# voidstrike/FPSG

Hardware: AMD Instinct MI355X
Metric: episodes/sec (+ Chamfer-kernel HBM GB/s in roofline.hbm), 2048-pt clouds, 224x224 images; episode = fwd + Chamfer + bwd, step = E episodes + all-reduce + Adam (higher is better)
Workload: dtype f32

## Files before the change

fpsg_amd/csrc/winograd_dw.hip:

```cpp
#include "fpsg_common.h"

namespace fpsg {
namespace {

constexpr int kDwThreads = 256;

__device__ __forceinline__ void in4(const float (&d)[6], float c0, float (&t)[6]) {
  const float p = fma_rn(-4.0f, d[2], d[4]), q = fma_rn(-4.0f, d[1], d[3]);
  const float r = d[4] - d[2], s = d[3] - d[1];
  t[0] = fma_rn(c0, d[0], fma_rn(-5.0f, d[2], d[4]));
  t[1] = p + q;
  t[2] = p - q;
  t[3] = fma_rn(2.0f, s, r);
  t[4] = fma_rn(-2.0f, s, r);
  t[5] = fma_rn(4.0f, d[1], fma_rn(-5.0f, d[3], d[5]));
}
__device__ __forceinline__ void gout4(const float (&y)[4], float (&r)[6]) {
  const float e = y[0] + y[2], o = y[1] + y[3];
  r[0] = y[0];
  r[1] = e + o;
  r[2] = e - o;
  const float e4 = fma_rn(4.0f, y[2], y[0]), o4 = fma_rn(8.0f, y[3], 2.0f * y[1]);
  r[3] = e4 + o4;
  r[4] = e4 - o4;
  r[5] = y[3];
}

constexpr int kXInstr = 36, kGInstr = 4;
constexpr int kStageFloats = (kXInstr + kGInstr) * 64 * 4;
constexpr int kDma = 10;

template <bool ACT>
__global__ __launch_bounds__(kDwThreads) void wino4_dw_c64_kernel(const float* __restrict__ x, const float* __restrict__ dy,
                                                                  int K, int H, int W, int Th, int Tw, int n_img,
                                                                  long n_steps, int KB, int spr,
                                                                  float* __restrict__ part ,
                                                                  const float* __restrict__ chan,
                                                                  const float* __restrict__ pre_bias) {
  constexpr int C = 64;
  extern __shared__ __attribute__((aligned(16))) float stage[];
  const int tid = threadIdx.x, lane = tid & 63;
  const int wave = __builtin_amdgcn_readfirstlane(tid >> 6);
  const int kk = lane >> 4, col = lane & 15;
  const int i = blockIdx.x;
  const int kb = (i >> 3) % KB;
  const int rg = (i & 7) + 8 * (i / (8 * KB));
  const long s0 = (long)rg * spr;
  const long s1 = (s0 + spr) < n_steps ? (s0 + spr) : n_steps;
  const int cx = wave * 16 + col;
  float* out = part + (((size_t)rg * 36) * K + kb * 16 + 4 * kk) * C + cx;
  if (s0 >= s1) {
#pragma unroll
    for (int xi = 0; xi < 36; ++xi)
#pragma unroll
      for (int r = 0; r < 4; ++r) out[((size_t)xi * K + r) * C] = 0.0f;
    return;
  }
  const __amdgpu_buffer_rsrc_t xrsrc = __builtin_amdgcn_make_buffer_rsrc(
      const_cast<float*>(x), 0, (int)((size_t)n_img * C * H * W * sizeof(float)), 0x00020000);
  const __amdgpu_buffer_rsrc_t grsrc = __builtin_amdgcn_make_buffer_rsrc(
      const_cast<float*>(dy), 0, (int)((size_t)n_img * K * H * W * sizeof(float)), 0x00020000);
  float asc = 1.0f, ash = 0.0f, apb = 0.0f;
  if (ACT) { asc = chan[cx]; ash = chan[C + cx]; apb = pre_bias ? pre_bias[cx] : 0.0f; }

  int fix[kDma];
  int rsel[9];
#pragma unroll
  for (int d = 0; d < 9; ++d) {
    const int p = (wave + 4 * d) * 64 + lane;
    const int r = p / 384, rem = p - r * 384, ch = rem / 6, q = rem - 6 * ch;
    rsel[d] = r;
    fix[d] = ch * H * W + 4 * q - 4;
  }
  {
    const int p = wave * 64 + lane, k = p >> 4, j = ((p & 15) - (k & 7)) & 15;
    fix[9] = ((kb * 16 + k) * H + (j >> 2)) * W + 4 * (j & 3);
  }
  int tw0, th;
  unsigned n;
  {
    const unsigned p0 = (unsigned)(4 * s0);
    tw0 = (int)(p0 % (unsigned)Tw);
    const unsigned q = p0 / (unsigned)Tw;
    th = (int)(q % (unsigned)Th);
    n = q / (unsigned)Th;
  }
  uint32_t rowoff[kDma];
  auto place_row = [&]() {
    const int r0 = 4 * th - 1;
    const int xbase = (int)(n * (unsigned)(C * H * W)), gbase = (int)(n * (unsigned)(K * H * W)) + 4 * th * W;
#pragma unroll
    for (int d = 0; d < 9; ++d) {
      const int row = r0 + rsel[d];
      rowoff[d] = (uint32_t)(xbase + fix[d] + (row < 0 ? 0 : (row >= H ? H - 1 : row)) * W) * 4u;
    }
    rowoff[9] = (uint32_t)(gbase + fix[9]) * 4u;
  };
  place_row();
  auto issue = [&](int buf) {
    const uint32_t cadv = (uint32_t)tw0 * 16u;
    float* sb = stage + buf * kStageFloats;
#pragma unroll
    for (int d = 0; d < 9; ++d)
      __builtin_amdgcn_raw_ptr_buffer_load_lds(xrsrc, (__attribute__((address_space(3))) void*)(sb + (wave + 4 * d) * 256), 16,
                                               rowoff[d] + cadv, 0, 0, 0);
    __builtin_amdgcn_raw_ptr_buffer_load_lds(grsrc, (__attribute__((address_space(3))) void*)(sb + (kXInstr + wave) * 256), 16,
                                             rowoff[9] + cadv, 0, 0, 0);
  };
  auto advance = [&]() {
    tw0 += 4;
    if (tw0 >= Tw) {
      tw0 = 0;
      if (++th >= Th) { th = 0; ++n; }
      place_row();
    }
  };
  v4f acc[36];
#pragma unroll
  for (int xi = 0; xi < 36; ++xi) acc[xi] = (v4f){0.0f, 0.0f, 0.0f, 0.0f};
  auto act = [&](float v) { return ACT ? __builtin_fmaxf(fma_rn(v + apb, asc, ash), 0.0f) : v; };
  int gslot[4];
#pragma unroll
  for (int a = 0; a < 4; ++a) gslot[a] = (4 * a + kk + (col & 7)) & 15;
  auto compute = [&](const float* sb, int tw, int thc, v4f (&accr)[36]) {
    const int r0 = 4 * thc - 1;
    const float c4t = r0 >= 0 ? 4.0f : 0.0f, mb = r0 + 5 < H ? 1.0f : 0.0f;
    const float c4l = tw > 0 ? 4.0f : 0.0f, mr = tw < Tw - 1 ? 1.0f : 0.0f, mr5 = mr * mb;
    const v4f* xs = reinterpret_cast<const v4f*>(sb) + cx * 6 + kk;
    float d[6][6];
#pragma unroll
    for (int r = 0; r < 6; ++r) {
      const v4f lf = xs[r * 384], md = xs[r * 384 + 1], rt = xs[r * 384 + 2];
      const float l = act(lf[3]), m0 = act(md[0]), m1 = act(md[1]), m2 = act(md[2]), m3 = act(md[3]), rr = act(rt[0]);
      d[r][0] = r == 5 ? l * mb : l;
      d[r][1] = r == 5 ? m0 * mb : m0;
      d[r][2] = r == 5 ? m1 * mb : m1;
      d[r][3] = r == 5 ? m2 * mb : m2;
      d[r][4] = r == 5 ? m3 * mb : m3;
      d[r][5] = rr * (r == 5 ? mr5 : mr);
    }
    float t[6][6];
#pragma unroll
    for (int j = 0; j < 6; ++j) {
      const float colv[6] = {d[0][j], d[1][j], d[2][j], d[3][j], d[4][j], d[5][j]};
      in4(colv, c4t, t[j]);
    }
    const v4f* gs = reinterpret_cast<const v4f*>(sb + kXInstr * 256) + col * 16;
    v4f g[4];
#pragma unroll
    for (int a = 0; a < 4; ++a) g[a] = gs[gslot[a]];
    float u[4][6];
#pragma unroll
    for (int j = 0; j < 4; ++j) {
      const float colv[4] = {g[0][j], g[1][j], g[2][j], g[3][j]};
      gout4(colv, u[j]);
    }
#pragma unroll
    for (int i2 = 0; i2 < 6; ++i2) {
      const float rowb[6] = {t[0][i2], t[1][i2], t[2][i2], t[3][i2], t[4][i2], t[5][i2]};
      const float rowa[4] = {u[0][i2], u[1][i2], u[2][i2], u[3][i2]};
      float ob[6], oa[6];
      in4(rowb, c4l, ob);
      gout4(rowa, oa);
      const int x0 = 6 * i2;
      asm volatile(
          "s_nop 1\n\t"
          "v_mfma_f32_16x16x4_f32 %0, %6, %12, %0\n\t"
          "v_mfma_f32_16x16x4_f32 %1, %7, %13, %1\n\t"
          "v_mfma_f32_16x16x4_f32 %2, %8, %14, %2\n\t"
          "v_mfma_f32_16x16x4_f32 %3, %9, %15, %3\n\t"
          "v_mfma_f32_16x16x4_f32 %4, %10, %16, %4\n\t"
          "v_mfma_f32_16x16x4_f32 %5, %11, %17, %5"
          : "+a"(accr[x0]), "+a"(accr[x0 + 1]), "+a"(accr[x0 + 2]), "+a"(accr[x0 + 3]), "+a"(accr[x0 + 4]),
            "+a"(accr[x0 + 5])
          : "v"(oa[0]), "v"(oa[1]), "v"(oa[2]), "v"(oa[3]), "v"(oa[4]), "v"(oa[5]),
            "v"(ob[0]), "v"(ob[1]), "v"(ob[2]), "v"(ob[3]), "v"(ob[4]), "v"(ob[5]));
    }
  };
  issue(0);
  __builtin_amdgcn_s_waitcnt(0);
  __syncthreads();
  int buf = 0;
  for (long s = s0; s < s1; ++s) {
    const int tw_now = tw0 + kk, th_now = th;
    if (s + 1 < s1) {
      advance();
      issue(buf ^ 1);
    }
    __builtin_amdgcn_sched_barrier(0);
    compute(stage + buf * kStageFloats, tw_now, th_now, acc);
    __builtin_amdgcn_sched_barrier(0);
    __builtin_amdgcn_s_waitcnt(0);
    __syncthreads();
    buf ^= 1;
  }
  asm volatile("s_nop 15\n\ts_nop 15" ::: "memory");
  __builtin_amdgcn_sched_barrier(0);
#pragma unroll
  for (int xi = 0; xi < 36; ++xi)
#pragma unroll
    for (int r = 0; r < 4; ++r) out[((size_t)xi * K + r) * C] = acc[xi][r];
}

__global__ __launch_bounds__(256) void wino_dw_reduce_kernel(const float* __restrict__ part, int R, long n,
                                                             float* __restrict__ dU) {
  const long e = (long)blockIdx.x * 256 + threadIdx.x;
  if (e >= n) return;
  double a = 0.0;
  for (int r = 0; r < R; ++r) a += (double)part[(size_t)r * n + e];
  dU[e] = (float)a;
}

long dw_ranges(int KB, long n_steps) {
  long cap = ((512 + KB - 1) / KB + 7) / 8 * 8;
  long want = ((n_steps + 31) / 32 + 7) / 8 * 8;
  return want < cap ? want : cap;
}

}
}

extern "C" size_t fpsg_wino_dw_fused_workspace_floats(int N, int K, int H, int W) {
  if (N <= 0 || K <= 0 || K % 16 || H <= 0 || W <= 0) return 0;
  if (H % 4 || W % 16) return 0;
  return (size_t)fpsg::dw_ranges(K / 16, (long)N * (H / 4) * (W / 4) / 4) * 36 * K * 64;
}

extern "C" int fpsg_wino_dw_fused(const float* x, const float* chan, const float* pre_bias, const float* dy, int N, int C,
                                  int K, int H, int W, float* dU, float* ws, fpsg_stream_t stream) {
  using namespace fpsg;
  const char* fn = "fpsg_wino_dw_fused";
  FPSG_REQUIRE(C == 64, FPSG_E_SHAPE, "%s: C must be 64 (got %d)", fn, C);
  FPSG_REQUIRE(N > 0 && K > 0 && K % 16 == 0 && K <= 1024 && H > 0 && W > 0 && H % 4 == 0 && W % 16 == 0, FPSG_E_SHAPE,
               "%s: K a positive multiple of 16 (<= 1024), H a multiple of 4 and W of 16 (four tiles per step lie "
               "in one tile row; got K=%d H=%d W=%d)", fn, K, H, W);
  FPSG_REQUIRE_PTR(x); FPSG_REQUIRE_PTR(dy); FPSG_REQUIRE_PTR(dU); FPSG_REQUIRE_PTR(ws);
  FPSG_REQUIRE(((reinterpret_cast<uintptr_t>(x) | reinterpret_cast<uintptr_t>(dy)) & 15) == 0, FPSG_E_ALIGN,
               "%s: x and dy must be 16-byte aligned", fn);
  FPSG_REQUIRE(!misaligned4(chan) && !misaligned4(pre_bias) && !misaligned4(dU) && !misaligned4(ws), FPSG_E_ALIGN,
               "%s: chan / pre_bias / dU / ws not 4-byte aligned", fn);
  FPSG_REQUIRE((size_t)N * (K > C ? K : C) * H * W * sizeof(float) < ((size_t)1 << 31), FPSG_E_LIMIT,
               "%s: x and dy must be below 2 GiB each (32-bit lane offsets; got N=%d K=%d H=%d W=%d)", fn, N, K, H, W);
  const int Th = H / 4, Tw = W / 4, KB = K / 16;
  const long n_steps = (long)N * Th * Tw / 4;
  const long R = dw_ranges(KB, n_steps);
  const int spr = (int)((n_steps + R - 1) / R);
  hipStream_t s = static_cast<hipStream_t>(stream);
  dim3 grid((unsigned)(R * KB));
  const size_t lds_bytes = 2 * (size_t)kStageFloats * sizeof(float);
  typedef void (*kern_t)(const float*, const float*, int, int, int, int, int, int, long, int, int, float*, const float*,
                         const float*);
  const kern_t kern = chan ? wino4_dw_c64_kernel<true> : wino4_dw_c64_kernel<false>;
  const hipError_t lds_optin = hipFuncSetAttribute(reinterpret_cast<const void*>(kern),
                                                   hipFuncAttributeMaxDynamicSharedMemorySize, 160 * 1024);
  if (lds_optin != hipSuccess) {
    set_error("%s: cannot reserve %zu B of LDS: %s", fn, lds_bytes, hipGetErrorString(lds_optin));
    return static_cast<int>(lds_optin);
  }
  hipLaunchKernelGGL(kern, grid, dim3(kDwThreads), lds_bytes, s, x, dy, K, H, W, Th, Tw, N, n_steps, KB, spr, ws, chan,
                     chan ? pre_bias : nullptr);
  int rc = launch_status(fn);
  if (rc) return rc;
  const long n = 36L * K * 64;
  hipLaunchKernelGGL(wino_dw_reduce_kernel, dim3((unsigned)((n + 255) / 256)), dim3(256), 0, s, ws, (int)R, n, dU);
  return launch_status("fpsg_wino_dw_fused(reduce)");
}
```

Baseline: 46.37.

## Add wide 32-output-channel Winograd weight-gradient kernel with triple-buffered loads

Adds a wide variant of the Winograd 4x4 depthwise-filter gradient kernel in which each block covers 32 output channels instead of 16. The transformed input tile is reused across two MFMA accumulator sets, and part of the second set is held in VGPRs rather than AGPRs. The staged DMA pipeline becomes triple-buffered and interleaves load issue with the MFMA groups. The aim is to halve the input-transform work and x loads per output channel and to hide load latency better. In exchange, register pressure and LDS use rise, and the grid has half as many blocks. It is enabled by default when K is a multiple of 32, and an environment variable can turn it off.

```diff
diff --git a/fpsg_amd/csrc/winograd_dw.hip b/fpsg_amd/csrc/winograd_dw.hip
--- a/fpsg_amd/csrc/winograd_dw.hip
+++ b/fpsg_amd/csrc/winograd_dw.hip
@@ -1,4 +1,7 @@
 #include "fpsg_common.h"
+
+#include <stdlib.h>
+#include <string.h>
 
 namespace fpsg {
 namespace {
@@ -202,6 +205,230 @@
     for (int r = 0; r < 4; ++r) out[((size_t)xi * K + r) * C] = acc[xi][r];
 }
 
+constexpr int kGInstrW = 8;
+constexpr int kStageFloatsW = (kXInstr + kGInstrW) * 64 * 4;
+constexpr int kDmaW = 11;
+constexpr int kBufsW = 3;
+constexpr int kWaitVm0 = 0x0F70, kWaitVm11 = 0x0F70 | kDmaW;
+
+#define FPSG_DW_MFMA6(CS, ACC, X0, OA, OB)                                                                          \
+  asm volatile(                                                                                                     \
+      "s_nop 1\n\t"                                                                                                 \
+      "v_mfma_f32_16x16x4_f32 %0, %6, %12, %0\n\t"                                                                  \
+      "v_mfma_f32_16x16x4_f32 %1, %7, %13, %1\n\t"                                                                  \
+      "v_mfma_f32_16x16x4_f32 %2, %8, %14, %2\n\t"                                                                  \
+      "v_mfma_f32_16x16x4_f32 %3, %9, %15, %3\n\t"                                                                  \
+      "v_mfma_f32_16x16x4_f32 %4, %10, %16, %4\n\t"                                                                 \
+      "v_mfma_f32_16x16x4_f32 %5, %11, %17, %5"                                                                     \
+      : "+" CS(ACC[X0]), "+" CS(ACC[X0 + 1]), "+" CS(ACC[X0 + 2]), "+" CS(ACC[X0 + 3]), "+" CS(ACC[X0 + 4]),        \
+        "+" CS(ACC[X0 + 5])                                                                                         \
+      : "v"(OA[0]), "v"(OA[1]), "v"(OA[2]), "v"(OA[3]), "v"(OA[4]), "v"(OA[5]),                                     \
+        "v"(OB[0]), "v"(OB[1]), "v"(OB[2]), "v"(OB[3]), "v"(OB[4]), "v"(OB[5]))
+
+template <bool ACT>
+__global__ __launch_bounds__(kDwThreads) void wino4_dw_c64_wide_kernel(const float* __restrict__ x,
+                                                                       const float* __restrict__ dy, int K, int H, int W,
+                                                                       int Th, int Tw, int n_img, long n_steps, int KB2,
+                                                                       int spr, float* __restrict__ part ,
+                                                                       const float* __restrict__ chan,
+                                                                       const float* __restrict__ pre_bias) {
+  constexpr int C = 64;
+  extern __shared__ __attribute__((aligned(16))) float stage[];
+  const int tid = threadIdx.x, lane = tid & 63;
+  const int wave = __builtin_amdgcn_readfirstlane(tid >> 6);
+  const int kk = lane >> 4, col = lane & 15;
+  const int i = blockIdx.x;
+  const int kb = (i >> 3) % KB2;
+  const int rg = (i & 7) + 8 * (i / (8 * KB2));
+  const long s0 = (long)rg * spr;
+  const long s1 = (s0 + spr) < n_steps ? (s0 + spr) : n_steps;
+  const int cx = wave * 16 + col;
+  float* out = part + (((size_t)rg * 36) * K + kb * 32 + 4 * kk) * C + cx;
+  if (s0 >= s1) {
+#pragma unroll
+    for (int xi = 0; xi < 36; ++xi)
+#pragma unroll
+      for (int r = 0; r < 4; ++r) {
+        out[((size_t)xi * K + r) * C] = 0.0f;
+        out[((size_t)xi * K + 16 + r) * C] = 0.0f;
+      }
+    return;
+  }
+  const __amdgpu_buffer_rsrc_t xrsrc = __builtin_amdgcn_make_buffer_rsrc(
+      const_cast<float*>(x), 0, (int)((size_t)n_img * C * H * W * sizeof(float)), 0x00020000);
+  const __amdgpu_buffer_rsrc_t grsrc = __builtin_amdgcn_make_buffer_rsrc(
+      const_cast<float*>(dy), 0, (int)((size_t)n_img * K * H * W * sizeof(float)), 0x00020000);
+  float asc = 1.0f, ash = 0.0f, apb = 0.0f;
+  if (ACT) { asc = chan[cx]; ash = chan[C + cx]; apb = pre_bias ? pre_bias[cx] : 0.0f; }
+
+  int tw0, th;
+  unsigned n;
+  {
+    const unsigned p0 = (unsigned)(4 * s0);
+    tw0 = (int)(p0 % (unsigned)Tw);
+    const unsigned q = p0 / (unsigned)Tw;
+    th = (int)(q % (unsigned)Th);
+    n = q / (unsigned)Th;
+  }
+  int ctw = tw0, cth = th;
+  uint32_t rowoff[kDmaW];
+  auto place_row = [&]() {
+    const int r0 = 4 * th - 1;
+    const int xbase = (int)(n * (unsigned)(C * H * W)), gbase = (int)(n * (unsigned)(K * H * W)) + 4 * th * W;
+#pragma unroll
+    for (int d = 0; d < 9; ++d) {
+      const int p = (wave + 4 * d) * 64 + lane;
+      const int r = p / 384, rem = p - r * 384, ch = rem / 6, q = rem - 6 * ch;
+      const int row = r0 + r;
+      rowoff[d] = (uint32_t)(xbase + ch * H * W + 4 * q - 4 + (row < 0 ? 0 : (row >= H ? H - 1 : row)) * W) * 4u;
+    }
+    const int p = wave * 64 + lane, k = p >> 4, j = ((p & 15) - (k & 7)) & 15;
+    rowoff[9] = (uint32_t)(gbase + ((kb * 32 + k) * H + (j >> 2)) * W + 4 * (j & 3)) * 4u;
+    rowoff[10] = rowoff[9] + (uint32_t)(16 * H * W) * 4u;
+  };
+  place_row();
+  auto issue1 = [&](float* sb, int d) {
+    const uint32_t cadv = (uint32_t)tw0 * 16u;
+    if (d < 9)
+      __builtin_amdgcn_raw_ptr_buffer_load_lds(xrsrc, (__attribute__((address_space(3))) void*)(sb + (wave + 4 * d) * 256), 16,
+                                               rowoff[d] + cadv, 0, 0, 0);
+    else
+      __builtin_amdgcn_raw_ptr_buffer_load_lds(grsrc,
+                                               (__attribute__((address_space(3))) void*)(sb + (kXInstr + 4 * (d - 9) + wave) * 256),
+                                               16, rowoff[d] + cadv, 0, 0, 0);
+  };
+  auto advance = [&]() {
+    tw0 += 4;
+    if (tw0 >= Tw) {
+      tw0 = 0;
+      if (++th >= Th) { th = 0; ++n; }
+      place_row();
+    }
+  };
+  v4f acc0[36], acc1[36];
+#pragma unroll
+  for (int xi = 0; xi < 36; ++xi) {
+    acc0[xi] = (v4f){0.0f, 0.0f, 0.0f, 0.0f};
+    acc1[xi] = (v4f){0.0f, 0.0f, 0.0f, 0.0f};
+  }
+  auto act = [&](float v) { return ACT ? __builtin_fmaxf(fma_rn(v + apb, asc, ash), 0.0f) : v; };
+  int gslot[4];
+#pragma unroll
+  for (int a = 0; a < 4; ++a) gslot[a] = (4 * a + kk + (col & 7)) & 15;
+
+#pragma unroll
+  for (int d = 0; d < kDmaW; ++d) issue1(stage, d);
+  if (s0 + 1 < s1) {
+    advance();
+#pragma unroll
+    for (int d = 0; d < kDmaW; ++d) issue1(stage + kStageFloatsW, d);
+  }
+  __builtin_amdgcn_s_waitcnt(0);
+  __builtin_amdgcn_s_barrier();
+  int cb = 0, db = 2;
+  for (long s = s0; s < s1; ++s) {
+    const bool pf = s + 2 < s1;
+    if (pf) advance();
+    const float* sb = stage + cb * kStageFloatsW;
+    float* sd = stage + db * kStageFloatsW;
+    __builtin_amdgcn_sched_barrier(0);
+    {
+      const int tw = ctw + kk;
+      const int r0 = 4 * cth - 1;
+      const float c4t = r0 >= 0 ? 4.0f : 0.0f, mb = r0 + 5 < H ? 1.0f : 0.0f;
+      const float c4l = tw > 0 ? 4.0f : 0.0f, mr = tw < Tw - 1 ? 1.0f : 0.0f, mr5 = mr * mb;
+      const float* xs = sb + (cx * 6 + kk) * 4;
+      float d[6][6];
+#pragma unroll
+      for (int r = 0; r < 6; ++r) {
+        const v4f md = *reinterpret_cast<const v4f*>(xs + r * 1536 + 4);
+        const float l = act(xs[r * 1536 + 3]), m0 = act(md[0]), m1 = act(md[1]), m2 = act(md[2]), m3 = act(md[3]),
+                    rr = act(xs[r * 1536 + 8]);
+        d[r][0] = r == 5 ? l * mb : l;
+        d[r][1] = r == 5 ? m0 * mb : m0;
+        d[r][2] = r == 5 ? m1 * mb : m1;
+        d[r][3] = r == 5 ? m2 * mb : m2;
+        d[r][4] = r == 5 ? m3 * mb : m3;
+        d[r][5] = rr * (r == 5 ? mr5 : mr);
+      }
+      float t[6][6];
+#pragma unroll
+      for (int j = 0; j < 6; ++j) {
+        const float colv[6] = {d[0][j], d[1][j], d[2][j], d[3][j], d[4][j], d[5][j]};
+        in4(colv, c4t, t[j]);
+      }
+      float u[2][4][6];
+#pragma unroll
+      for (int h = 0; h < 2; ++h) {
+        const v4f* gs = reinterpret_cast<const v4f*>(sb + (kXInstr + 4 * h) * 256) + col * 16;
+        v4f g[4];
+#pragma unroll
+        for (int a = 0; a < 4; ++a) g[a] = gs[gslot[a]];
+#pragma unroll
+        for (int j = 0; j < 4; ++j) {
+          const float colv[4] = {g[0][j], g[1][j], g[2][j], g[3][j]};
+          gout4(colv, u[h][j]);
+        }
+      }
+#pragma unroll
+      for (int i2 = 0; i2 < 6; ++i2) {
+        const float rowb[6] = {t[0][i2], t[1][i2], t[2][i2], t[3][i2], t[4][i2], t[5][i2]};
+        float ob[6];
+        in4(rowb, c4l, ob);
+        const int x0 = 6 * i2;
+        {
+          const float rowa[4] = {u[0][0][i2], u[0][1][i2], u[0][2][i2], u[0][3][i2]};
+          float oa[6];
+          gout4(rowa, oa);
+          FPSG_DW_MFMA6("a", acc0, x0, oa, ob);
+        }
+        __builtin_amdgcn_sched_barrier(0);
+        if (pf) issue1(sd, 2 * i2);
+        __builtin_amdgcn_sched_barrier(0);
+        {
+          const float rowa[4] = {u[1][0][i2], u[1][1][i2], u[1][2][i2], u[1][3][i2]};
+          float oa[6];
+          gout4(rowa, oa);
+          if (i2 < 4) FPSG_DW_MFMA6("a", acc1, x0, oa, ob);
+          else        FPSG_DW_MFMA6("v", acc1, x0, oa, ob);
+        }
+        __builtin_amdgcn_sched_barrier(0);
+        if (i2 < 5) {
+          if (pf) issue1(sd, 2 * i2 + 1);
+          __builtin_amdgcn_sched_barrier(0);
+        }
+      }
+    }
+    if (pf) __builtin_amdgcn_s_waitcnt(kWaitVm11);
+    else    __builtin_amdgcn_s_waitcnt(kWaitVm0);
+    __builtin_amdgcn_s_barrier();
+    cb = cb == kBufsW - 1 ? 0 : cb + 1;
+    db = db == kBufsW - 1 ? 0 : db + 1;
+    ctw += 4;
+    if (ctw >= Tw) {
+      ctw = 0;
+      if (++cth >= Th) cth = 0;
+    }
+  }
+  asm volatile("s_nop 15\n\ts_nop 15" ::: "memory");
+  __builtin_amdgcn_sched_barrier(0);
+#pragma unroll
+  for (int xi = 0; xi < 36; ++xi) {
+#pragma unroll
+    for (int r = 0; r < 4; ++r) {
+      out[((size_t)xi * K + r) * C] = acc0[xi][r];
+      out[((size_t)xi * K + 16 + r) * C] = acc1[xi][r];
+    }
+    if (xi + 1 < 36) {
+      asm volatile("" : "+a"(acc0[xi + 1]) : : "memory");
+      if (xi + 1 < 24) asm volatile("" : "+a"(acc1[xi + 1]) : : "memory");
+      else             asm volatile("" : "+v"(acc1[xi + 1]) : : "memory");
+    }
+  }
+}
+#undef FPSG_DW_MFMA6
+static_assert(kDmaW == 11, "the counted wait of the wide kernel's step names the number of loads per wave and step");
+
 __global__ __launch_bounds__(256) void wino_dw_reduce_kernel(const float* __restrict__ part, int R, long n,
                                                              float* __restrict__ dU) {
   const long e = (long)blockIdx.x * 256 + threadIdx.x;
@@ -215,6 +442,11 @@
   long cap = ((512 + KB - 1) / KB + 7) / 8 * 8;
   long want = ((n_steps + 31) / 32 + 7) / 8 * 8;
   return want < cap ? want : cap;
+}
+
+bool dw_wide(int K) {
+  const char* e = getenv("FPSG_K6W_WIDE");
+  return K % 32 == 0 && !(e != nullptr && strcmp(e, "0") == 0);
 }
 
 }
@@ -246,19 +478,22 @@
   const long R = dw_ranges(KB, n_steps);
   const int spr = (int)((n_steps + R - 1) / R);
   hipStream_t s = static_cast<hipStream_t>(stream);
-  dim3 grid((unsigned)(R * KB));
-  const size_t lds_bytes = 2 * (size_t)kStageFloats * sizeof(float);
+  const bool wide = dw_wide(K);
+  const int blocks = wide ? KB / 2 : KB;
+  dim3 grid((unsigned)(R * blocks));
+  const size_t lds_bytes = (wide ? kBufsW * (size_t)kStageFloatsW : 2 * (size_t)kStageFloats) * sizeof(float);
   typedef void (*kern_t)(const float*, const float*, int, int, int, int, int, int, long, int, int, float*, const float*,
                          const float*);
   const kern_t kern = chan ? wino4_dw_c64_kernel<true> : wino4_dw_c64_kernel<false>;
-  const hipError_t lds_optin = hipFuncSetAttribute(reinterpret_cast<const void*>(kern),
+  const kern_t launch = !wide ? kern : chan ? wino4_dw_c64_wide_kernel<true> : wino4_dw_c64_wide_kernel<false>;
+  const hipError_t lds_optin = hipFuncSetAttribute(reinterpret_cast<const void*>(launch),
                                                    hipFuncAttributeMaxDynamicSharedMemorySize, 160 * 1024);
   if (lds_optin != hipSuccess) {
     set_error("%s: cannot reserve %zu B of LDS: %s", fn, lds_bytes, hipGetErrorString(lds_optin));
     return static_cast<int>(lds_optin);
   }
-  hipLaunchKernelGGL(kern, grid, dim3(kDwThreads), lds_bytes, s, x, dy, K, H, W, Th, Tw, N, n_steps, KB, spr, ws, chan,
-                     chan ? pre_bias : nullptr);
+  hipLaunchKernelGGL(launch, grid, dim3(kDwThreads), lds_bytes, s, x, dy, K, H, W, Th, Tw, N, n_steps, blocks, spr, ws,
+                     chan, chan ? pre_bias : nullptr);
   int rc = launch_status(fn);
   if (rc) return rc;
   const long n = 36L * K * 64;
```

New measurement: 46.14, median of 2. Within noise of the previous version (-0.5%).
